# maxgillett/tinysplat

Hardware: AMD Instinct MI355X
Metric: Gaussians*pixels/s fwd+bwd (higher is better)
Workload: dtype f32; 1 GPU; 1000000 random Gaussians, SH degree 3, 1920x1080, fwd+bwd (RGB), BASELINE configs[2]; max_per_tile=614, parallelism=single GPU, tile_lists=16x16 (gsplat's) (auto), gaussian_order=as generated (i.i.d.)

## Files before the change

include/tinysplat_hip.h:

```cpp
#ifndef TINYSPLAT_HIP_H
#define TINYSPLAT_HIP_H

#include <stdint.h>

#ifdef __cplusplus
extern "C" {
#endif

#define TS_ABI_VERSION 8

#define TS_E_BADARG (-1)
#define TS_E_DEGREE (-2)

#define TS_TILE 16
#define TS_SPLAT_RECORD_FLOATS 12
#define TS_PARTIAL_ROW_FLOATS 12

int ts_abi_version(void);

typedef struct ts_camera {
    float fx, fy, cx, cy;
    int32_t img_width, img_height;
    int32_t tile_bounds_x, tile_bounds_y;
    int32_t tile_row0, tile_rows;
// ... 60 lines not shown
                    const int32_t* cum_tiles_hit, int64_t capacity, void* stream);
int ts_tile_offsets_stats(int32_t n, int32_t num_tiles, int32_t* bin_ws, int32_t* tile_bins,
                          const int32_t* cum_tiles_hit, int64_t capacity, int32_t* longest_list, void* stream);

int ts_bin_scatter(int32_t n, const float* xys, const int32_t* radii, const float* splats,
                   const ts_camera* cam_host, const int32_t* bin_ws, int32_t* bucket_ids, int32_t* scratch,
                   void* stream);

int ts_sort_tiles(int32_t num_tiles, const int32_t* tile_bins, const float* depths,
                  const int32_t* bucket_ids, int32_t* gaussian_ids_sorted, int32_t* sort_ws,
                  int32_t* zeroed_counter, void* stream);
int ts_sort_tiles_above(int32_t num_tiles, const int32_t* tile_bins, const float* depths,
                        const int32_t* bucket_ids, int32_t* gaussian_ids_sorted, int32_t* sort_ws,
                        int32_t* zeroed_counter, void* stream);

#define TS_RASTER_LOGIT_OPACITY 1

int ts_pack_splats(int32_t n, int32_t channels, int32_t flags, const float* xys, const int32_t* radii,
                   const float* conics, const float* colors, const float* opacity,
                   const int32_t* cum_tiles_hit, const ts_camera* cam_host, const float* depths,
                   float* splats, void* stream);

#define TS_RASTER_CLAMP_RGB 2
#define TS_RASTER_SPLIT_BLOCKS 4
#define TS_RASTER_NARROW_WAVES 8
#define TS_RASTER_FLAG_GEN(g) (((g) & 0xff) << 8)
int ts_raster_fwd(int32_t channels, int32_t flags, const ts_camera* cam_host, const int32_t* tile_bins,
                  const int32_t* gaussian_ids_sorted, const float* splats, const float* background,
                  float* out_img, float* final_Ts, int32_t* final_index, uint8_t* clamp_mask,
                  void* stream);
// ... 21 lines not shown

int ts_reduce_partials(int32_t n, int32_t channels, int32_t flags, const int32_t* num_tiles_hit,
                       const int32_t* cum_tiles_hit, const float* partials,
                       const uint8_t* row_flags, const float* splats, float* v_xy, float* v_conic,
                       float* v_colors, float* v_opacity, float* v_depth, const uint8_t* color_mask,
                       void* stream);

#define TS_FRAME_TIGHT 1
#define TS_FRAME_SPLIT 2
#define TS_FRAME_NARROW_WAVES 8
#define TS_FRAME_DIRECT_SCATTER 32
#define TS_FRAME_PLANES 64
#define TS_FRAME_LIST_STATS 256
#define TS_FRAME_SEPARATE_SORT 128
#define TS_FRAME_STRIPE 16
#define TS_FRAME_SURVIVORS 512
typedef struct ts_frame {
    int32_t n, num_bases, sh_degree, channels, flags;
    int32_t flag_gen;
    ts_camera cam;
    const float *means, *scales, *quats, *opacities, *colors_dc, *colors_rest;
    const float *view34, *projview, *origin, *background;
    float *xys, *depths, *conics, *colors, *splats;
    int32_t *radii, *num_tiles_hit, *cum_tiles_hit;
    uint8_t* sh_mask;
    int32_t *scan_ws, *bin_ws, *tile_bins;
    int32_t* total_host;
    int64_t num_intersects;
    int64_t capacity;
    int32_t *bucket_ids, *gaussian_ids_sorted;
// ... 285 lines not shown
```

tinysplat_amd/_lib.py:

```python
from __future__ import annotations

import ctypes
import os
from ctypes import POINTER, c_double, c_float, c_int32, c_int64, c_void_p
from pathlib import Path

LIB_PATH = Path(os.environ["TS_LIB_PATH"]) if os.environ.get("TS_LIB_PATH") else \
    Path(__file__).resolve().parent / "csrc" / "libtinysplat_hip.so"
ABI_VERSION = 8
HINT_BALANCED_WALK = 1
HINT_COOP_SPLIT = 1 << 20
PARTIAL_ROW_FLOATS = 12


class TsCamera(ctypes.Structure):
    _fields_ = [
        ("fx", c_float), ("fy", c_float), ("cx", c_float), ("cy", c_float),
        ("img_width", c_int32), ("img_height", c_int32),
        ("tile_bounds_x", c_int32), ("tile_bounds_y", c_int32),
        ("tile_row0", c_int32), ("tile_rows", c_int32),
        ("glob_scale", c_float), ("clip_thresh", c_float),
        ("wide_tiles", c_int32), ("hints", c_int32),
    ]

# ... 60 lines not shown
    "ts_project_fwd": (c_int32, [c_int32, _P, _P, _P, _P, _P, _CAM, c_int32, _P, _P, _P, _P, _P, _P, _P]),
    "ts_project_bwd": (c_int32, [c_int32, _P, _P, _P, _P, _P, _CAM, c_int32, _P, _P, _P, _P, _P, _P, _P, _P, _P]),
    "ts_sh_fwd": (c_int32, [c_int32, c_int32, c_int32, _P, _P, _P, _P]),
    "ts_sh_bwd": (c_int32, [c_int32, c_int32, c_int32, _P, _P, _P, _P]),
    "ts_sh_colors_fwd": (c_int32, [c_int32, c_int32, c_int32, _P, _P, _P, _P, _P, _P, _P, _P]),
    "ts_sh_colors_bwd": (c_int32, [c_int32, c_int32, c_int32, _P, _P, _P, _P, _P, _P, _P]),
    "ts_scan_ws_ints": (c_int64, [c_int32]),
    "ts_scan_tiles": (c_int32, [c_int32, _P, _P, _P, _P, _P]),
    "ts_bin_ws_ints": (c_int64, [c_int32, c_int32]),
    "ts_bin_count": (c_int32, [c_int32, _P, _P, _P, _CAM, _P, _P]),
    "ts_tile_offsets": (c_int32, [c_int32, c_int32, _P, _P, _P, c_int64, _P]),
    "ts_tile_offsets_stats": (c_int32, [c_int32, c_int32, _P, _P, _P, c_int64, _P, _P]),
    "ts_bin_scatter": (c_int32, [c_int32, _P, _P, _P, _CAM, _P, _P, _P, _P]),
    "ts_sort_tiles": (c_int32, [c_int32, _P, _P, _P, _P, _P, _P, _P]),
    "ts_sort_tiles_above": (c_int32, [c_int32, _P, _P, _P, _P, _P, _P, _P]),
    "ts_num_tiles": (c_int32, [_CAM]),
    "ts_final_floats": (c_int64, [_CAM, c_int32]),
    "ts_cut_tiles": (c_int32, [_CAM, _P, _P]),
    "ts_colors_pack_fwd": (c_int32, [c_int32, c_int32, c_int32, _P, _P, _P, _P, _P, _P, c_int32, c_int32,
                                     _P, _P, _P, _P, _P, _CAM, _P, _P, _P]),
    "ts_pack_splats": (c_int32, [c_int32, c_int32, c_int32, _P, _P, _P, _P, _P, _P, _CAM, _P, _P, _P]),
    "ts_raster_fwd": (c_int32, [c_int32, c_int32, _CAM, _P, _P, _P, _P, _P, _P, _P, _P, _P]),
    "ts_raster_bwd": (c_int32, [c_int32, c_int32, c_int64, _CAM, _P, _P, _P, _P, _P, _P, _P, _P, _P, _P, _P, _P]),
    "ts_raster_fwd_planes": (c_int32, [c_int32, c_int32, _CAM, _P, _P, _P, _P, _P, _P, _P, _P, _P, _P]),
    "ts_raster_fwd_sort": (c_int32, [c_int32, c_int32, _CAM, _P, _P, _P, _P, _P, _P, _P, _P, _P, _P, _P, _P]),
    "ts_raster_bwd_planes": (c_int32, [c_int32, c_int32, c_int64, _CAM, _P, _P, _P, _P, _P, _P, _P, _P, c_int32,
                                       _P, _P, _P, _P, _P]),
    "ts_bench_stream_read": (c_int32, [_P, c_int64, _P, _P]),
    "ts_bench_gather48": (c_int32, [_P, _P, c_int64, _P, _P]),
    "ts_photometric_ws_floats": (c_int64, [c_int32, c_int32]),
# ... 140 lines not shown
```

tinysplat_amd/csrc/binning.hip:

```cpp
#include <hip/hip_runtime.h>

#include "../../include/tinysplat_hip.h"
#include "host_util.h"
#include "pack.h"
#include "splat_math.h"

namespace {

constexpr int kThreads = 256;
constexpr int kScanItems = 4;
constexpr int kScanBlock = kThreads * kScanItems;

__device__ __forceinline__ int wave_inclusive_scan(int v) {
    const int lane = threadIdx.x & 63;
#pragma unroll
    for (int d = 1; d < 64; d <<= 1) {
        const int u = __shfl_up(v, d, 64);
        if (lane >= d) v += u;
    }
    return v;
}

template <int WAVES = 4>
__device__ __forceinline__ int block_inclusive_scan(int v, int* total) {
// ... 374 lines not shown
        t -= t0;
        if ((unsigned)t < (unsigned)tw) bucket_ids[atomicAdd(&cursor[t], 1)] = i;
    });
}

#ifndef TS_COARSE_SHIFT
#define TS_COARSE_SHIFT 5
#endif
constexpr int kCoarseShift = TS_COARSE_SHIFT;
constexpr int kCoarseTiles = 1 << kCoarseShift;
constexpr int kCoarseIdBits = 32 - kCoarseShift;
#ifndef TS_TWO_HOP_FROM
#define TS_TWO_HOP_FROM (1 << 18)
#endif
constexpr int kTwoHopFrom = TS_TWO_HOP_FROM;

template <bool BAL>
__global__ __launch_bounds__(kBinThreads) void bin_scatter_coarse_kernel(
    int n, int chunk, const float* __restrict__ xys, const int* __restrict__ radii,
    const float4* __restrict__ splats, const ts_camera cam, int num_tiles, const int* __restrict__ bases,
    const int* __restrict__ tile_start, int* __restrict__ scratch) {
    extern __shared__ int cursor[];
    if (tile_start[num_tiles + 1] != 0) return;
    const int groups = (num_tiles + kCoarseTiles - 1) >> kCoarseShift;
    const int* src = bases + (size_t)blockIdx.x * num_tiles;
    for (int g = threadIdx.x; g < groups; g += kBinThreads) cursor[g] = tile_start[g << kCoarseShift];
    __syncthreads();
    for (int t = threadIdx.x; t < num_tiles; t += kBinThreads) {
        const int v = src[t];
        if (v) atomicAdd(&cursor[t >> kCoarseShift], v);
    }
    __syncthreads();
    const int g0 = blockIdx.x * chunk, g1 = min(n, g0 + chunk);
    auto emit = [&](int t, int i) {
        scratch[atomicAdd(&cursor[t >> kCoarseShift], 1)] = i | ((t & (kCoarseTiles - 1)) << kCoarseIdBits);
    };
    if (BAL) walk_chunk_balanced(g0, g1, xys, radii, splats, cam, emit);
    else walk_chunk(g0, g1, xys, radii, splats, cam, emit);
}

#ifndef TS_FINE_THREADS
#define TS_FINE_THREADS 1024
#endif
#ifndef TS_FINE_AHEAD
#define TS_FINE_AHEAD 8
// ... 57 lines not shown
            }
        }
        __syncthreads();
#pragma unroll
        for (int u = 0; u < kFineAhead; ++u) {
            const int k = u * kFineThreads + (int)threadIdx.x;
            if (k < m) {
                const int t = tiles[k];
                bucket_ids[gbase[t] + (k - loff[t])] = ids[k];
            }
        }
        __syncthreads();
    }
}

constexpr int kSortCap = 4096;

#include "sort_network.h"

struct IdKeyArray {
    volatile int* ids;
    const float* depths;
};

__device__ __forceinline__ void cmpswap(IdKeyArray a, int i, int j) {
    const int x = a.ids[i], y = a.ids[j];
    if (make_key(a.depths, x) > make_key(a.depths, y)) { a.ids[i] = y; a.ids[j] = x; }
}

template <typename Ptr>
// ... 140 lines not shown
        const int s0 = start[b], m = start[b + 1] - s0;
        __syncthreads();
        if (m <= kSortCap) {
            sort_bucket_block(out + s0, depths, out + s0, m, scratch);
        } else {
            IdKeyArray a{out + s0, depths};
            bitonic_network(a, m);
        }
        __syncthreads();
    }
}

__global__ __launch_bounds__(kThreads) void sort_tiles_small_kernel(
    int num_tiles, const int* __restrict__ tile_bins, const float* __restrict__ depths,
    const int* __restrict__ bucket_ids, int* __restrict__ ids_sorted, int* __restrict__ large_count,
    int* __restrict__ large_list) {
    const int lane = threadIdx.x & 63;
    const int tile = blockIdx.x * (kThreads / 64) + (threadIdx.x >> 6);
    if (tile >= num_tiles) return;
    const int2 range = reinterpret_cast<const int2*>(tile_bins)[tile];
    const int n = range.y - range.x;
    if (n <= 0) return;
    if (n > kWaveSortMax) {
        if (n > kSortCap && lane == 0) large_list[atomicAdd(large_count, 1)] = tile;
        return;
    }
    const int* g = bucket_ids + range.x;
    int* out = ids_sorted + range.x;
    if (n <= 64) sort_tile_wave<1>(g, depths, out, n, lane);
    else if (n <= 128) sort_tile_wave<2>(g, depths, out, n, lane);
    else if (n <= 256) sort_tile_wave<4>(g, depths, out, n, lane);
// ... 18 lines not shown
    const int* __restrict__ bucket_ids, int* __restrict__ ids_sorted,
    const int* __restrict__ large_count, const int* __restrict__ large_list) {
    __shared__ unsigned long long lds_large[kLargeLdsU64];
    const int count = *large_count;
    for (int q = blockIdx.x; q < count; q += gridDim.x) {
        const int2 range = reinterpret_cast<const int2*>(tile_bins)[large_list[q]];
        const int n = range.y - range.x;
        if (n <= kSortCap) continue;
        __syncthreads();
        sort_tile_sample(bucket_ids + range.x, depths, ids_sorted + range.x, n, lds_large);
    }
}

__global__ __launch_bounds__(kThreads) void sort_tiles_above_kernel(
    const int* __restrict__ tile_bins, const float* __restrict__ depths,
    const int* __restrict__ bucket_ids, int* __restrict__ ids_sorted) {
    __shared__ unsigned long long lds_u64[kLargeLdsU64 > kSortCap / 2 ? kLargeLdsU64 : kSortCap / 2];
    const int2 range = reinterpret_cast<const int2*>(tile_bins)[blockIdx.x];
    const int n = range.y - range.x;
    if (n <= kWaveSortMax) return;
    if (n <= kSortCap) sort_bucket_block(bucket_ids + range.x, depths, ids_sorted + range.x, n, lds_u64);
    else sort_tile_sample(bucket_ids + range.x, depths, ids_sorted + range.x, n, lds_u64);
}

__global__ __launch_bounds__(kThreads) void pack_splats_kernel(int n, const ts::PackArgs a,
                                                              const float* __restrict__ colors) {
    const int i = blockIdx.x * kThreads + threadIdx.x;
    if (i >= n) return;
    if (a.radii[i] <= 0) return;
    float c0, c1, c2, c3 = 0.0f;
    if (a.channels == 4 && a.depths == nullptr) {
        const float4 c = reinterpret_cast<const float4*>(colors)[i];
// ... 71 lines not shown
    if (n < 0 || num_tiles < 0) return TS_E_BADARG;
    if (num_tiles == 0) return 0;
    if (!bin_ws || !tile_bins) return TS_E_BADARG;
    const int chunks = bin_num_chunks(n);
    int* tile_total = bin_ws + (size_t)chunks * num_tiles;
    const int per_group = (chunks + kScanGroups - 1) / kScanGroups;
    hipStream_t s = (hipStream_t)stream;
    hipLaunchKernelGGL(column_scan_kernel, dim3((num_tiles + kColTiles - 1) / kColTiles),
                       dim3(kColTiles * kScanGroups), 0, s, num_tiles, chunks, per_group, bin_ws, tile_total);
    hipLaunchKernelGGL(tile_offsets_kernel, dim3(1), dim3(kOffsetsThreads), 0, s, num_tiles, tile_total,
                       tile_bins, bin_ws + (ts_bin_ws_ints(n, num_tiles) - 1),
                       (cum_tiles_hit && n > 0) ? cum_tiles_hit + (n - 1) : nullptr, (long long)capacity, longest_list);
    return launch_status();
}

int ts_bin_scatter(int32_t n, const float* xys, const int32_t* radii, const float* splats,
                   const ts_camera* cam, const int32_t* bin_ws, int32_t* bucket_ids, int32_t* scratch,
                   void* stream) {
    if (n < 0 || !cam) return TS_E_BADARG;
    if (n == 0) return 0;
    if (!xys || !radii || !bin_ws || !bucket_ids) return TS_E_BADARG;
    const int nt = ts_num_tiles(cam);
    if (nt <= 0) return 0;
    const int chunks = bin_num_chunks(n);
    const int chunk = (n + chunks - 1) / chunks;
    const int* tile_start = bin_ws + (size_t)chunks * nt;
    if (scratch && n >= kTwoHopFrom && n < (1 << kCoarseIdBits)) {
        const int groups = (nt + kCoarseTiles - 1) >> kCoarseShift;
        if (cam->hints & TS_HINT_BALANCED_WALK)
            hipLaunchKernelGGL(bin_scatter_coarse_kernel<true>, dim3(chunks), dim3(kBinThreads),
                               (size_t)groups * sizeof(int), (hipStream_t)stream, n, chunk, xys, radii,
                               reinterpret_cast<const float4*>(splats), *cam, nt, bin_ws, tile_start, scratch);
        else
            hipLaunchKernelGGL(bin_scatter_coarse_kernel<false>, dim3(chunks), dim3(kBinThreads),
                               (size_t)groups * sizeof(int), (hipStream_t)stream, n, chunk, xys, radii,
                               reinterpret_cast<const float4*>(splats), *cam, nt, bin_ws, tile_start, scratch);
        hipLaunchKernelGGL(bin_scatter_fine_kernel, dim3(groups), dim3(kFineThreads), 0, (hipStream_t)stream, nt,
                           tile_start, scratch, bucket_ids);
        return launch_status();
    }
    const int window = bin_window_tiles(n, nt);
    const int windows = (nt + window - 1) / window;
    const size_t lds = (size_t)window * sizeof(int);
    if (lds > 64 * 1024)
        (void)hipFuncSetAttribute(reinterpret_cast<const void*>(&bin_scatter_kernel),
                                  hipFuncAttributeMaxDynamicSharedMemorySize, (int)lds);
    hipLaunchKernelGGL(bin_scatter_kernel, dim3(chunks, windows), dim3(kBinThreads), lds,
                       (hipStream_t)stream, n, chunk, xys, radii,
                       reinterpret_cast<const float4*>(splats), *cam, nt, window, bin_ws,
                       tile_start, bucket_ids);
    return launch_status();
}

int ts_sort_tiles(int32_t num_tiles, const int32_t* tile_bins, const float* depths,
                  const int32_t* bucket_ids, int32_t* gaussian_ids_sorted, int32_t* sort_ws,
                  int32_t* zeroed_counter, void* stream) {
    if (num_tiles < 0) return TS_E_BADARG;
    if (num_tiles == 0) return 0;
    if (!tile_bins || !depths || !bucket_ids || !gaussian_ids_sorted || !sort_ws) return TS_E_BADARG;
    hipStream_t s = (hipStream_t)stream;
    int32_t* counter = zeroed_counter ? zeroed_counter : sort_ws;
    int32_t* list = zeroed_counter ? sort_ws : sort_ws + 1;
    if (!zeroed_counter) {
        hipError_t e = hipMemsetAsync(sort_ws, 0, sizeof(int32_t), s);
        if (e != hipSuccess) return (int)e;
    }
    hipLaunchKernelGGL(sort_tiles_small_kernel, dim3((num_tiles + kThreads / 64 - 1) / (kThreads / 64)),
                       dim3(kThreads), 0, s, (int)num_tiles, tile_bins, depths, bucket_ids,
                       gaussian_ids_sorted, counter, list);
    hipLaunchKernelGGL(sort_tiles_mid_kernel, dim3(num_tiles), dim3(kThreads), 0, s, tile_bins, depths,
                       bucket_ids, gaussian_ids_sorted, (int*)nullptr, (int*)nullptr);
    const int grid = num_tiles < 768 ? num_tiles : 768;
    hipLaunchKernelGGL(sort_tiles_large_kernel, dim3(grid), dim3(kThreads), 0, s, tile_bins, depths,
                       bucket_ids, gaussian_ids_sorted, counter, list);
    return launch_status();
}

int ts_sort_tiles_above(int32_t num_tiles, const int32_t* tile_bins, const float* depths,
                        const int32_t* bucket_ids, int32_t* gaussian_ids_sorted, int32_t* sort_ws,
                        int32_t* zeroed_counter, void* stream) {
    if (num_tiles < 0) return TS_E_BADARG;
    if (num_tiles == 0) return 0;
    if (!tile_bins || !depths || !bucket_ids || !gaussian_ids_sorted) return TS_E_BADARG;
    (void)sort_ws; (void)zeroed_counter;
    hipLaunchKernelGGL(sort_tiles_above_kernel, dim3(num_tiles), dim3(kThreads), 0, (hipStream_t)stream, tile_bins,
                       depths, bucket_ids, gaussian_ids_sorted);
    return launch_status();
}

int ts_pack_splats(int32_t n, int32_t channels, int32_t flags, const float* xys, const int32_t* radii,
                   const float* conics, const float* colors, const float* opacity,
                   const int32_t* cum_tiles_hit, const ts_camera* cam, const float* depths, float* splats,
                   void* stream) {
    if (n < 0 || !cam || (channels != 3 && channels != 4)) return TS_E_BADARG;
    if (n == 0) return 0;
    if (!xys || !radii || !conics || !colors || !opacity || !cum_tiles_hit || !splats)
        return TS_E_BADARG;
    ts::PackArgs a;
    a.channels = channels; a.flags = (int)flags; a.xys = xys; a.radii = radii; a.conics = conics;
    a.opacity = opacity; a.cum_tiles_hit = cum_tiles_hit; a.depths = depths;
    a.splats = reinterpret_cast<float4*>(splats); a.cam = *cam;
// ... 7 lines not shown
```

tinysplat_amd/csrc/frame.hip:

```cpp
#include <hip/hip_runtime.h>

#include <atomic>
#include <cstdlib>
#if !defined(TS_NO_ROCTX) && __has_include(<rocprofiler-sdk-roctx/roctx.h>)
#include <rocprofiler-sdk-roctx/roctx.h>
#define TS_HAVE_ROCTX 1
#else
#define TS_HAVE_ROCTX 0
#endif

#include "../../include/tinysplat_hip.h"
#include "raster_survivors.h"

struct TsRange {
#if TS_HAVE_ROCTX
    explicit TsRange(const char* name) { roctxRangePush(name); }
    ~TsRange() { roctxRangePop(); }
#else
    explicit TsRange(const char*) {}
#endif
};

static std::atomic<ts_entry_probe> g_probe{nullptr};
static std::atomic<void*> g_probe_user{nullptr};
// ... 48 lines not shown
}
inline int bwd_split(const ts_frame* f) {
    return ((f->flags & TS_FRAME_SPLIT) && !segmented(f)) ? TS_RASTER_SPLIT_BLOCKS : 0;
}
inline int small_n_fused() {
    static const int v = [] {
        const char* e = getenv("TS_SMALL_N_FUSED");
        return e ? atoi(e) : 262144;
    }();
    return v;
}
inline bool survivors(const ts_frame* f) {
    return (f->flags & TS_FRAME_SURVIVORS) && f->survivors && f->final_Ts && f->num_intersects > 0 &&
           f->cam.wide_tiles == 0 &&
           !(f->flags & (TS_FRAME_SPLIT | TS_FRAME_NARROW_WAVES | TS_FRAME_SEPARATE_SORT));
}
inline int raster_flags(const ts_frame* f) {
    return TS_RASTER_CLAMP_RGB | ((f->flags & TS_FRAME_SPLIT) ? TS_RASTER_SPLIT_BLOCKS : 0) |
           ((f->flags & TS_FRAME_NARROW_WAVES) ? TS_RASTER_NARROW_WAVES : 0);
}
}

extern "C" {

int32_t ts_frame_struct_bytes(void) { return (int32_t)sizeof(ts_frame); }

int ts_set_entry_probe(ts_entry_probe fn, void* user) {
    g_probe_user.store(user, std::memory_order_relaxed);
    g_probe.store(fn, std::memory_order_release);
    return 0;
// ... 15 lines not shown
    }
    return 0;
}

int ts_frame_fwd_prepare(const ts_frame* f, void* stream) {
    TsRange range_("ts_frame_fwd_prepare");
    if (bad(f)) return TS_E_BADARG;
    TS_TRY(TS_ENTRY("ts_colors_pack_fwd",
                    ts_colors_pack_fwd(f->n, f->sh_degree, f->num_bases, f->means, f->origin, f->colors_dc,
                                       f->num_bases > 1 ? f->colors_rest : nullptr, f->sh_mask,
                                       (f->flags & TS_FRAME_STRIPE) ? f->num_tiles_hit : nullptr, f->channels,
                                       TS_RASTER_LOGIT_OPACITY, f->xys, f->radii, f->conics, f->opacities,
                                       f->cum_tiles_hit, &f->cam, f->channels == 4 ? f->depths : nullptr, f->splats,
                                       stream)));
    const float* tight = (f->flags & TS_FRAME_TIGHT) ? f->splats : nullptr;
    TS_TRY(TS_ENTRY("ts_bin_count", ts_bin_count(f->n, f->xys, f->radii, tight, &f->cam, f->bin_ws, stream)));
    int32_t* longest = nullptr;
    if ((f->flags & TS_FRAME_LIST_STATS) && f->total_host) {
        int32_t* dev = mapped_pointer(f->total_host);
        if (dev) longest = dev + 1;
    }
    TS_TRY(TS_ENTRY("ts_tile_offsets",
                    ts_tile_offsets_stats(f->n, num_tiles(f), f->bin_ws, f->tile_bins, f->cum_tiles_hit, f->capacity,
                                          longest, stream)));
    return 0;
}

int ts_frame_fwd_composite(const ts_frame* f, void* stream) {
    TsRange range_("ts_frame_fwd_composite");
    if (bad(f) || f->num_intersects < 0) return TS_E_BADARG;
    const bool planes = (f->flags & TS_FRAME_PLANES) != 0;
    if (planes && (f->channels != 4 || !f->out_depth)) return TS_E_BADARG;
    const bool fused_sort = f->num_intersects > 0 && f->cam.wide_tiles == 0 &&
                            !(f->flags & (TS_FRAME_NARROW_WAVES | TS_FRAME_SEPARATE_SORT));
    if (f->num_intersects > 0) {
        const float* tight = (f->flags & TS_FRAME_TIGHT) ? f->splats : nullptr;
        TS_TRY(TS_ENTRY("ts_bin_scatter",
                        ts_bin_scatter(f->n, f->xys, f->radii, tight, &f->cam, f->bin_ws, f->bucket_ids,
                                       (f->flags & TS_FRAME_DIRECT_SCATTER) ? nullptr : f->gaussian_ids_sorted,
                                       stream)));
        int32_t* counter = f->bin_ws + (ts_bin_ws_ints(f->n, num_tiles(f)) - 1);
        if (fused_sort)
            TS_TRY(TS_ENTRY("ts_sort_tiles",
                            ts_sort_tiles_above(num_tiles(f), f->tile_bins, f->depths, f->bucket_ids,
                                                f->gaussian_ids_sorted, f->bin_ws, counter, stream)));
        else
            TS_TRY(TS_ENTRY("ts_sort_tiles",
                            ts_sort_tiles(num_tiles(f), f->tile_bins, f->depths, f->bucket_ids, f->gaussian_ids_sorted,
                                          f->bin_ws, counter, stream)));
    }
    if (fused_sort)
        return TS_ENTRY("ts_raster_fwd",
                        ts_surv::raster_fwd_sort(f->channels, raster_flags(f), &f->cam, f->tile_bins, f->bucket_ids,
                                                 f->depths, f->gaussian_ids_sorted, f->splats, f->background,
                                                 f->out_img, planes ? f->out_depth : nullptr, f->final_Ts,
                                                 f->final_index, f->clamp_mask, survivors(f) ? f->survivors : nullptr,
                                                 stream));
    return TS_ENTRY("ts_raster_fwd",
                    ts_raster_fwd_planes(f->channels, raster_flags(f), &f->cam, f->tile_bins, f->gaussian_ids_sorted,
                                         f->splats, f->background, f->out_img, planes ? f->out_depth : nullptr,
                                         f->final_Ts, f->final_index, f->clamp_mask, stream));
}

int ts_frame_bwd_composite(const ts_frame* f, void* stream) {
// ... 185 lines not shown
```

tinysplat_amd/frame.py:

```python
from __future__ import annotations

import ctypes
import os
import threading
from typing import Optional, Tuple

import torch
import torch.distributed as dist
from torch import Tensor

from ._comm import collective_timer
from . import _lib
from ._lib import TsFrame
from .ops import TileBinning, _camera, _f32c, _need_hip, _stream, _stripe_rows, _tile_bounds, deg_from_sh

TIGHT_BINNING = os.environ.get("TS_TIGHT_BINNING", "1") != "0"

SPLIT_BLOCKS_BELOW = int(os.environ.get("TS_SPLIT_BLOCKS_BELOW", "2400"))

_ls = os.environ.get("TS_LIST_SEGMENTS", "auto")
LIST_SEGMENTS = _ls if _ls == "auto" else max(1, min(8, int(_ls)))
LIST_SEGMENTS_FROM = int(os.environ.get("TS_LIST_SEGMENTS_FROM", "192"))
SEGMENT_ITEMS = int(os.environ.get("TS_SEGMENT_ITEMS", "16384"))

# ... 128 lines not shown
        if slot[1] > 255:
            slot[0].zero_()
            slot[1] = 1
        return slot[0], slot[1]

_bg_cache = {}

STRIPE_SPARSE = os.environ.get("TS_STRIPE_SPARSE", "1") != "0"

TWO_HOP_SCATTER = os.environ.get("TS_TWO_HOP_SCATTER", "1") != "0"
INLINE_SORT = os.environ.get("TS_INLINE_SORT", "1") != "0"

DIRECT_GRADS = os.environ.get("TS_DIRECT_GRADS", "1") != "0"

SURVIVORS = os.environ.get("TS_SURVIVORS", "1") != "0"

CAPACITY_ALLOC = os.environ.get("TS_CAPACITY_ALLOC", "0") != "0"
CAPACITY_GROWTH = 1.25
_capacity = {}

COUNT_WAIT = os.environ.get("TS_COUNT_WAIT", "spin")
_SPIN_LIMIT = 50_000_000


def alloc_quantum(count: int) -> int:
    count = max(int(count), 1)
    if count <= 65536:
        return 65536
    g = 1 << (count.bit_length() - 4)
    return (count + g - 1) // g * g
# ... 100 lines not shown
        F.radii = view(5, torch.int32, n, (n,))
        F.nth = view(6, torch.int32, n, (n,))
        F.cum = view(7, torch.int32, n, (n,))
        F.tile_bins = view(10, torch.int32, 2 * max(num_tiles, 1), (max(num_tiles, 1), 2))
        host, event, count_lock = _total_slot(dev)
        fr = TsFrame()
        fr.n, fr.num_bases, fr.sh_degree, fr.channels = n, nb, int(sh_degree), ch
        stripe = STRIPE_SPARSE and cam.tile_rows < cam.tile_bounds_y
        full = cam.tile_rows == cam.tile_bounds_y
        fr.flags = ((1 if TIGHT_BINNING else 0) | (2 if F.split else 0) | (8 if mode == 2 else 0) | (16 if stripe else 0)
                    | (0 if TWO_HOP_SCATTER else 32) | (64 if F.planes else 0) | (0 if INLINE_SORT else 128)
                    | (256 if full else 0))
        surv = SURVIVORS and keep and full and mode == 0 and not F.split and INLINE_SORT
        if surv:
            fr.flags |= 512
        if full:
            _stats_mode[dev.index] = mode
        fr.cam = cam
        fr.means, fr.scales, fr.quats, fr.opacities = means.data_ptr(), scales.data_ptr(), quats.data_ptr(), opacities.data_ptr()
        fr.colors_dc, fr.colors_rest = colors_dc.data_ptr(), colors_rest.data_ptr()
        fr.view34, fr.projview, fr.origin, fr.background = view34.data_ptr(), projview.data_ptr(), origin.data_ptr(), bg.data_ptr()
        fr.splats, fr.xys, fr.conics, fr.depths = ptr[0], ptr[1], ptr[2], ptr[4]
        fr.radii, fr.num_tiles_hit, fr.cum_tiles_hit, fr.scan_ws = ptr[5], ptr[6], ptr[7], ptr[8]
        fr.bin_ws, fr.tile_bins = ptr[9], ptr[10]
        fr.total_host = host.data_ptr()
        fr.out_img = F.out_img.data_ptr()
        if F.planes:
            fr.out_depth = F.out_depth.data_ptr()
        if keep:
            fr.sh_mask, fr.final_Ts, fr.final_index, fr.clamp_mask = ptr[11], ptr[12], ptr[13], ptr[14]
# ... 242 lines not shown
```

Baseline: 2011000 billion Gaussians*pixels/s.

## Bin with per-group counts instead of per-tile counts in two-hop scatter

Adds a group-level binning path: the count kernel builds per-chunk histograms over coarse tile groups instead of every tile, a new offsets kernel scans those smaller chunk-by-group matrices, and a fine scatter kernel derives per-tile offsets and tile_bins inside each group. The longest-list statistic is now computed from per-group maxima inside the sort kernels. This cuts the size of the count workspace and the offset scan, at the cost of an extra per-group histogram pass in the fine scatter and more code paths.

```diff
diff --git a/include/tinysplat_hip.h b/include/tinysplat_hip.h
--- a/include/tinysplat_hip.h
+++ b/include/tinysplat_hip.h
@@ -98,6 +98,22 @@
                         const int32_t* bucket_ids, int32_t* gaussian_ids_sorted, int32_t* sort_ws,
                         int32_t* zeroed_counter, void* stream);
 
+int32_t ts_bin_group_form(int32_t n);
+int ts_bin_count_groups(int32_t n, const float* xys, const int32_t* radii, const float* splats,
+                        const ts_camera* cam_host, int32_t* bin_ws, void* stream);
+int ts_group_offsets(int32_t n, int32_t num_tiles, int32_t* bin_ws, int32_t* tile_bins,
+                     const int32_t* cum_tiles_hit, int64_t capacity, int32_t* longest_list, void* stream);
+int ts_bin_scatter_groups(int32_t n, const float* xys, const int32_t* radii, const float* splats,
+                          const ts_camera* cam_host, int32_t* bin_ws, int32_t* tile_bins, int32_t* bucket_ids,
+                          int32_t* scratch, void* stream);
+int ts_sort_tiles_stats(int32_t num_tiles, const int32_t* tile_bins, const float* depths,
+                        const int32_t* bucket_ids, int32_t* gaussian_ids_sorted, int32_t* sort_ws,
+                        int32_t* zeroed_counter, int32_t n, const int32_t* bin_ws, int32_t* longest_list,
+                        void* stream);
+int ts_sort_tiles_above_stats(int32_t num_tiles, const int32_t* tile_bins, const float* depths,
+                              const int32_t* bucket_ids, int32_t* gaussian_ids_sorted, int32_t n,
+                              const int32_t* bin_ws, int32_t* longest_list, void* stream);
+
 #define TS_RASTER_LOGIT_OPACITY 1
 
 int ts_pack_splats(int32_t n, int32_t channels, int32_t flags, const float* xys, const int32_t* radii,
@@ -149,6 +165,7 @@
 #define TS_FRAME_LIST_STATS 256
 #define TS_FRAME_SEPARATE_SORT 128
 #define TS_FRAME_STRIPE 16
+#define TS_FRAME_GROUP_COUNTS 1024
 #define TS_FRAME_SURVIVORS 512
 typedef struct ts_frame {
     int32_t n, num_bases, sh_degree, channels, flags;
diff --git a/tinysplat_amd/_lib.py b/tinysplat_amd/_lib.py
--- a/tinysplat_amd/_lib.py
+++ b/tinysplat_amd/_lib.py
@@ -98,6 +98,12 @@
     "ts_bin_scatter": (c_int32, [c_int32, _P, _P, _P, _CAM, _P, _P, _P, _P]),
     "ts_sort_tiles": (c_int32, [c_int32, _P, _P, _P, _P, _P, _P, _P]),
     "ts_sort_tiles_above": (c_int32, [c_int32, _P, _P, _P, _P, _P, _P, _P]),
+    "ts_bin_group_form": (c_int32, [c_int32]),
+    "ts_bin_count_groups": (c_int32, [c_int32, _P, _P, _P, _CAM, _P, _P]),
+    "ts_group_offsets": (c_int32, [c_int32, c_int32, _P, _P, _P, c_int64, _P, _P]),
+    "ts_bin_scatter_groups": (c_int32, [c_int32, _P, _P, _P, _CAM, _P, _P, _P, _P, _P]),
+    "ts_sort_tiles_stats": (c_int32, [c_int32, _P, _P, _P, _P, _P, _P, c_int32, _P, _P, _P]),
+    "ts_sort_tiles_above_stats": (c_int32, [c_int32, _P, _P, _P, _P, c_int32, _P, _P, _P]),
     "ts_num_tiles": (c_int32, [_CAM]),
     "ts_final_floats": (c_int64, [_CAM, c_int32]),
     "ts_cut_tiles": (c_int32, [_CAM, _P, _P]),
diff --git a/tinysplat_amd/csrc/binning.hip b/tinysplat_amd/csrc/binning.hip
--- a/tinysplat_amd/csrc/binning.hip
+++ b/tinysplat_amd/csrc/binning.hip
@@ -412,8 +412,110 @@
 #define TS_TWO_HOP_FROM (1 << 18)
 #endif
 constexpr int kTwoHopFrom = TS_TWO_HOP_FROM;
-
-template <bool BAL>
+inline bool two_hop(int n) { return n >= kTwoHopFrom && n < (1 << kCoarseIdBits); }
+static_assert(kTwoHopFrom >= 4096, "the group form's workspace layout needs bin_num_chunks(n) >= 4");
+
+__global__ __launch_bounds__(kBinThreads) void group_bin_count_kernel(
+    int n, int chunk, const float* __restrict__ xys, const int* __restrict__ radii,
+    const float4* __restrict__ splats, const ts_camera cam, int groups, int* __restrict__ counts) {
+    extern __shared__ int hist[];
+    for (int j = threadIdx.x; j < groups; j += kBinThreads) hist[j] = 0;
+    __syncthreads();
+    const int g0 = blockIdx.x * chunk, g1 = min(n, g0 + chunk);
+    walk_chunk(g0, g1, xys, radii, splats, cam, [&](int t, int) { atomicAdd(&hist[t >> kCoarseShift], 1); });
+    __syncthreads();
+    int* dst = counts + (size_t)blockIdx.x * groups;
+    for (int j = threadIdx.x; j < groups; j += kBinThreads) dst[j] = hist[j];
+}
+
+constexpr int kGoThreads = 1024;
+constexpr int kGoCols = 256;
+constexpr int kGoRows = kGoThreads / kGoCols;
+constexpr int kGoPer = 64;
+constexpr int kGoLdsGroups = 2048;
+constexpr int kGoSingleMax = 1 << 17;
+__global__ __launch_bounds__(kGoThreads) void group_tile_offsets_kernel(
+    int num_tiles, int groups, int chunks, int* __restrict__ counts, const int* col_total,
+    int* __restrict__ tile_start, int* __restrict__ tile_bins, int* __restrict__ spare,
+    const int* __restrict__ total_ptr, long long capacity, int* __restrict__ longest_out) {
+    __shared__ int rsum[kGoRows][kGoCols];
+    __shared__ int gtot[kGoLdsGroups];
+    __shared__ int carry, over;
+    const int tid = threadIdx.x;
+    if (tid == 0) {
+        carry = 0;
+        *spare = 0;
+        over = (total_ptr && capacity >= 0 && ((long long)*total_ptr > capacity || *total_ptr < 0)) ? 1 : 0;
+        spare[-1] = over;
+    }
+    __syncthreads();
+    if (!over) {
+        const int* tot = col_total;
+        if (counts) {
+            const int gl = tid & (kGoCols - 1), r = tid / kGoCols;
+#pragma unroll 1
+            for (int c0 = 0; c0 < groups; c0 += kGoCols) {
+                const int g = c0 + gl;
+                int colbase = 0;
+#pragma unroll 1
+                for (int r0 = 0; r0 < chunks; r0 += kGoRows * kGoPer) {
+                    const int b0 = r0 + r * kGoPer;
+                    int c[kGoPer];
+                    int sum = 0;
+                    const unsigned int col = (unsigned int)(b0 * groups + g);
+                    if (g < groups) {
+#pragma unroll
+                        for (int j = 0; j < kGoPer; ++j) c[j] = (b0 + j < chunks) ? counts[col + (unsigned int)(j * groups)] : 0;
+#pragma unroll
+                        for (int j = 0; j < kGoPer; ++j) {
+                            const int v = c[j];
+                            c[j] = sum;
+                            sum += v;
+                        }
+                    }
+                    rsum[r][gl] = sum;
+                    __syncthreads();
+                    int base = colbase, all = 0;
+#pragma unroll
+                    for (int q = 0; q < kGoRows; ++q) {
+                        const int v = rsum[q][gl];
+                        if (q < r) base += v;
+                        all += v;
+                    }
+                    if (g < groups) {
+#pragma unroll
+                        for (int j = 0; j < kGoPer; ++j)
+                            if (b0 + j < chunks) counts[col + (unsigned int)(j * groups)] = base + c[j];
+                    }
+                    colbase += all;
+                    __syncthreads();
+                }
+                if (r == 0 && g < groups) gtot[g] = colbase;
+            }
+            __syncthreads();
+            tot = gtot;
+        }
+        for (int base = 0; base < groups; base += kGoThreads) {
+            const int g = base + tid;
+            const int v = g < groups ? tot[g] : 0;
+            int total;
+            const int inc = block_inclusive_scan<kGoThreads / 64>(v, &total);
+            if (g < groups) tile_start[g << kCoarseShift] = carry + inc - v;
+            __syncthreads();
+            if (tid == 0) carry += total;
+            __syncthreads();
+        }
+        if (tid == 0) tile_start[num_tiles] = carry;
+        if (carry != 0) return;
+        if (tid == 0 && longest_out) *longest_out = 0;
+    }
+    for (int t = tid; t <= num_tiles; t += kGoThreads) {
+        tile_start[t] = 0;
+        if (t < num_tiles) reinterpret_cast<int2*>(tile_bins)[t] = make_int2(0, 0);
+    }
+}
+
+template <bool BAL, bool GROUPS = false>
 __global__ __launch_bounds__(kBinThreads) void bin_scatter_coarse_kernel(
     int n, int chunk, const float* __restrict__ xys, const int* __restrict__ radii,
     const float4* __restrict__ splats, const ts_camera cam, int num_tiles, const int* __restrict__ bases,
@@ -421,12 +523,17 @@
     extern __shared__ int cursor[];
     if (tile_start[num_tiles + 1] != 0) return;
     const int groups = (num_tiles + kCoarseTiles - 1) >> kCoarseShift;
-    const int* src = bases + (size_t)blockIdx.x * num_tiles;
-    for (int g = threadIdx.x; g < groups; g += kBinThreads) cursor[g] = tile_start[g << kCoarseShift];
-    __syncthreads();
-    for (int t = threadIdx.x; t < num_tiles; t += kBinThreads) {
-        const int v = src[t];
-        if (v) atomicAdd(&cursor[t >> kCoarseShift], v);
+    if (GROUPS) {
+        const int* src = bases + (size_t)blockIdx.x * groups;
+        for (int g = threadIdx.x; g < groups; g += kBinThreads) cursor[g] = tile_start[g << kCoarseShift] + src[g];
+    } else {
+        const int* src = bases + (size_t)blockIdx.x * num_tiles;
+        for (int g = threadIdx.x; g < groups; g += kBinThreads) cursor[g] = tile_start[g << kCoarseShift];
+        __syncthreads();
+        for (int t = threadIdx.x; t < num_tiles; t += kBinThreads) {
+            const int v = src[t];
+            if (v) atomicAdd(&cursor[t >> kCoarseShift], v);
+        }
     }
     __syncthreads();
     const int g0 = blockIdx.x * chunk, g1 = min(n, g0 + chunk);
@@ -514,6 +621,142 @@
     }
 }
 
+__global__ __launch_bounds__(kFineThreads) void bin_scatter_fine_groups_kernel(int num_tiles,
+                                                                               int* __restrict__ tile_start,
+                                                                               int* __restrict__ tile_bins,
+                                                                               int* __restrict__ group_max,
+                                                                               const int* __restrict__ scratch,
+                                                                               int* __restrict__ bucket_ids) {
+    if (tile_start[num_tiles + 1] != 0) return;
+    __shared__ int cursor[kCoarseTiles];
+    const int t0 = blockIdx.x << kCoarseShift, t1 = min(num_tiles, t0 + kCoarseTiles);
+    const int begin = tile_start[t0], end = tile_start[t1];
+    __shared__ int hist[kCoarseTiles], loff[kCoarseTiles + 1], gbase[kCoarseTiles];
+    __shared__ int ids[kFinePass];
+    __shared__ unsigned char tiles[kFinePass];
+    if ((int)threadIdx.x < kCoarseTiles) {
+        hist[threadIdx.x] = 0;
+        cursor[threadIdx.x] = 0;
+    }
+    __syncthreads();
+    auto publish = [&](int t, int c, int ex) {
+        const int s = begin + ex;
+        if (t < t1 - t0) {
+            cursor[t] = s;
+            if (t > 0) tile_start[t0 + t] = s;
+            reinterpret_cast<int2*>(tile_bins)[t0 + t] = c > 0 ? make_int2(s, s + c) : make_int2(0, 0);
+        }
+        int longest = c;
+#pragma unroll
+        for (int d = 32; d >= 1; d >>= 1) longest = max(longest, __shfl_xor(longest, d, 64));
+        if (t == 0) group_max[blockIdx.x] = longest;
+    };
+    const bool counted = end - begin > kFinePass || end == begin;
+    if (counted) {
+        for (int c0 = begin; c0 < end; c0 += kFinePass) {
+            const int m = min(kFinePass, end - c0);
+            unsigned int w[kFineAhead];
+#pragma unroll
+            for (int u = 0; u < kFineAhead; ++u) {
+                const int k = u * kFineThreads + (int)threadIdx.x;
+                if (k < m) w[u] = (unsigned int)scratch[c0 + k];
+            }
+#pragma unroll
+            for (int u = 0; u < kFineAhead; ++u) {
+                const int k = u * kFineThreads + (int)threadIdx.x;
+                if (k < m) atomicAdd(&hist[w[u] >> kCoarseIdBits], 1);
+            }
+        }
+        __syncthreads();
+        if ((int)threadIdx.x < 64) {
+            const int t = threadIdx.x;
+            const int c = t < kCoarseTiles ? hist[t] : 0;
+            int inc = c;
+#pragma unroll
+            for (int d = 1; d < kCoarseTiles; d <<= 1) {
+                const int o = __shfl_up(inc, d, 64);
+                if (t >= d) inc += o;
+            }
+            publish(t, c, inc - c);
+            if (t < kCoarseTiles) hist[t] = 0;
+        }
+        __syncthreads();
+    }
+    for (int c0 = begin; c0 < end; c0 += kFinePass) {
+        const int m = min(kFinePass, end - c0);
+        unsigned int w[kFineAhead];
+        int rank[kFineAhead];
+#pragma unroll
+        for (int u = 0; u < kFineAhead; ++u) {
+            const int k = u * kFineThreads + (int)threadIdx.x;
+            if (k < m) w[u] = (unsigned int)scratch[c0 + k];
+        }
+#pragma unroll
+        for (int u = 0; u < kFineAhead; ++u) {
+            const int k = u * kFineThreads + (int)threadIdx.x;
+            if (k < m) rank[u] = atomicAdd(&hist[w[u] >> kCoarseIdBits], 1);
+        }
+        __syncthreads();
+        if ((int)threadIdx.x < 64) {
+            const int t = threadIdx.x;
+            const int c = t < kCoarseTiles ? hist[t] : 0;
+            int inc = c;
+#pragma unroll
+            for (int d = 1; d < kCoarseTiles; d <<= 1) {
+                const int o = __shfl_up(inc, d, 64);
+                if (t >= d) inc += o;
+            }
+            if (!counted) publish(t, c, inc - c);
+            if (t < kCoarseTiles) {
+                loff[t] = inc - c;
+                gbase[t] = cursor[t];
+                cursor[t] += c;
+                hist[t] = 0;
+            }
+        }
+        __syncthreads();
+#pragma unroll
+        for (int u = 0; u < kFineAhead; ++u) {
+            const int k = u * kFineThreads + (int)threadIdx.x;
+            if (k < m) {
+                const int t = (int)(w[u] >> kCoarseIdBits);
+                const int lp = loff[t] + rank[u];
+                ids[lp] = (int)(w[u] & ((1u << kCoarseIdBits) - 1u));
+                tiles[lp] = (unsigned char)t;
+            }
+        }
+        __syncthreads();
+#pragma unroll
+        for (int u = 0; u < kFineAhead; ++u) {
+            const int k = u * kFineThreads + (int)threadIdx.x;
+            if (k < m) {
+                const int t = tiles[k];
+                bucket_ids[gbase[t] + (k - loff[t])] = ids[k];
+            }
+        }
+        __syncthreads();
+    }
+}
+
+struct ListStats {
+    const int* group_max;
+    const int* guard;
+    int* longest_out;
+    int groups;
+};
+__device__ __forceinline__ void store_longest(const ListStats& st) {
+    __shared__ int longest;
+    if (threadIdx.x == 0) longest = 0;
+    __syncthreads();
+    int m = 0;
+    for (int g = threadIdx.x; g < st.groups; g += kThreads) m = max(m, st.group_max[g]);
+#pragma unroll
+    for (int d = 32; d >= 1; d >>= 1) m = max(m, __shfl_xor(m, d, 64));
+    if ((threadIdx.x & 63) == 0) atomicMax(&longest, m);
+    __syncthreads();
+    if (threadIdx.x == 0 && *st.guard == 0) *st.longest_out = longest;
+}
+
 constexpr int kSortCap = 4096;
 
 #include "sort_network.h"
@@ -684,7 +927,8 @@
 __global__ __launch_bounds__(kThreads) void sort_tiles_small_kernel(
     int num_tiles, const int* __restrict__ tile_bins, const float* __restrict__ depths,
     const int* __restrict__ bucket_ids, int* __restrict__ ids_sorted, int* __restrict__ large_count,
-    int* __restrict__ large_list) {
+    int* __restrict__ large_list, const ListStats stats) {
+    if (stats.group_max && blockIdx.x == 0) store_longest(stats);
     const int lane = threadIdx.x & 63;
     const int tile = blockIdx.x * (kThreads / 64) + (threadIdx.x >> 6);
     if (tile >= num_tiles) return;
@@ -733,8 +977,9 @@
 
 __global__ __launch_bounds__(kThreads) void sort_tiles_above_kernel(
     const int* __restrict__ tile_bins, const float* __restrict__ depths,
-    const int* __restrict__ bucket_ids, int* __restrict__ ids_sorted) {
+    const int* __restrict__ bucket_ids, int* __restrict__ ids_sorted, const ListStats stats) {
     __shared__ unsigned long long lds_u64[kLargeLdsU64 > kSortCap / 2 ? kLargeLdsU64 : kSortCap / 2];
+    if (stats.group_max && blockIdx.x == 0) store_longest(stats);
     const int2 range = reinterpret_cast<const int2*>(tile_bins)[blockIdx.x];
     const int n = range.y - range.x;
     if (n <= kWaveSortMax) return;
@@ -836,6 +1081,76 @@
     return launch_status();
 }
 
+int32_t ts_bin_group_form(int32_t n) { return two_hop(n) ? 1 : 0; }
+
+int ts_bin_count_groups(int32_t n, const float* xys, const int32_t* radii, const float* splats,
+                        const ts_camera* cam, int32_t* bin_ws, void* stream) {
+    if (!cam || !bin_ws || !xys || !radii || !two_hop(n)) return TS_E_BADARG;
+    const int nt = ts_num_tiles(cam);
+    if (nt <= 0) return 0;
+    const int chunks = bin_num_chunks(n);
+    const int chunk = (n + chunks - 1) / chunks;
+    const int groups = (nt + kCoarseTiles - 1) >> kCoarseShift;
+    hipLaunchKernelGGL(group_bin_count_kernel, dim3(chunks), dim3(kBinThreads), (size_t)groups * sizeof(int),
+                       (hipStream_t)stream, n, chunk, xys, radii, reinterpret_cast<const float4*>(splats), *cam,
+                       groups, bin_ws);
+    return launch_status();
+}
+
+int ts_group_offsets(int32_t n, int32_t num_tiles, int32_t* bin_ws, int32_t* tile_bins,
+                     const int32_t* cum_tiles_hit, int64_t capacity, int32_t* longest_list, void* stream) {
+    if (num_tiles < 0 || !two_hop(n)) return TS_E_BADARG;
+    if (num_tiles == 0) return 0;
+    if (!bin_ws || !tile_bins) return TS_E_BADARG;
+    const int chunks = bin_num_chunks(n);
+    const int groups = (num_tiles + kCoarseTiles - 1) >> kCoarseShift;
+    int* tile_start = bin_ws + (size_t)chunks * num_tiles;
+    int* spare = bin_ws + (ts_bin_ws_ints(n, num_tiles) - 1);
+    const int* total_ptr = cum_tiles_hit ? cum_tiles_hit + (n - 1) : nullptr;
+    hipStream_t s = (hipStream_t)stream;
+    if ((long long)chunks * groups <= kGoSingleMax && groups <= kGoLdsGroups) {
+        hipLaunchKernelGGL(group_tile_offsets_kernel, dim3(1), dim3(kGoThreads), 0, s, num_tiles, groups, chunks,
+                           bin_ws, (const int*)nullptr, tile_start, tile_bins, spare, total_ptr, (long long)capacity,
+                           longest_list);
+    } else {
+        int* col_total = bin_ws + (size_t)chunks * groups;
+        const int per_group = (chunks + kScanGroups - 1) / kScanGroups;
+        hipLaunchKernelGGL(column_scan_kernel, dim3((groups + kColTiles - 1) / kColTiles),
+                           dim3(kColTiles * kScanGroups), 0, s, groups, chunks, per_group, bin_ws, col_total);
+        hipLaunchKernelGGL(group_tile_offsets_kernel, dim3(1), dim3(kGoThreads), 0, s, num_tiles, groups, chunks,
+                           (int*)nullptr, (const int*)col_total, tile_start, tile_bins, spare, total_ptr,
+                           (long long)capacity, longest_list);
+    }
+    return launch_status();
+}
+
+int ts_bin_scatter_groups(int32_t n, const float* xys, const int32_t* radii, const float* splats,
+                          const ts_camera* cam, int32_t* bin_ws, int32_t* tile_bins, int32_t* bucket_ids,
+                          int32_t* scratch, void* stream) {
+    if (!cam || !xys || !radii || !bin_ws || !tile_bins || !bucket_ids || !scratch || !two_hop(n))
+        return TS_E_BADARG;
+    const int nt = ts_num_tiles(cam);
+    if (nt <= 0) return 0;
+    const int chunks = bin_num_chunks(n);
+    const int chunk = (n + chunks - 1) / chunks;
+    const int groups = (nt + kCoarseTiles - 1) >> kCoarseShift;
+    int* tile_start = bin_ws + (size_t)chunks * nt;
+    hipStream_t s = (hipStream_t)stream;
+    if (cam->hints & TS_HINT_BALANCED_WALK)
+        hipLaunchKernelGGL((bin_scatter_coarse_kernel<true, true>), dim3(chunks), dim3(kBinThreads),
+                           (size_t)groups * sizeof(int), s, n, chunk, xys, radii,
+                           reinterpret_cast<const float4*>(splats), *cam, nt, (const int*)bin_ws,
+                           (const int*)tile_start, scratch);
+    else
+        hipLaunchKernelGGL((bin_scatter_coarse_kernel<false, true>), dim3(chunks), dim3(kBinThreads),
+                           (size_t)groups * sizeof(int), s, n, chunk, xys, radii,
+                           reinterpret_cast<const float4*>(splats), *cam, nt, (const int*)bin_ws,
+                           (const int*)tile_start, scratch);
+    hipLaunchKernelGGL(bin_scatter_fine_groups_kernel, dim3(groups), dim3(kFineThreads), 0, s, nt, tile_start,
+                       tile_bins, bin_ws + nt + 1, (const int*)scratch, bucket_ids);
+    return launch_status();
+}
+
 int ts_bin_scatter(int32_t n, const float* xys, const int32_t* radii, const float* splats,
                    const ts_camera* cam, const int32_t* bin_ws, int32_t* bucket_ids, int32_t* scratch,
                    void* stream) {
@@ -847,7 +1162,7 @@
     const int chunks = bin_num_chunks(n);
     const int chunk = (n + chunks - 1) / chunks;
     const int* tile_start = bin_ws + (size_t)chunks * nt;
-    if (scratch && n >= kTwoHopFrom && n < (1 << kCoarseIdBits)) {
+    if (scratch && two_hop(n)) {
         const int groups = (nt + kCoarseTiles - 1) >> kCoarseShift;
         if (cam->hints & TS_HINT_BALANCED_WALK)
             hipLaunchKernelGGL(bin_scatter_coarse_kernel<true>, dim3(chunks), dim3(kBinThreads),
@@ -874,12 +1189,39 @@
     return launch_status();
 }
 
+}
+
+namespace {
+inline bool list_stats(int n, int num_tiles, const int32_t* bin_ws, int32_t* longest_list, ListStats* st) {
+    *st = ListStats{nullptr, nullptr, nullptr, 0};
+    if (!longest_list) return true;
+    if (!bin_ws || !two_hop(n) || num_tiles <= 0) return false;
+    st->group_max = bin_ws + num_tiles + 1;
+    st->guard = bin_ws + (size_t)bin_num_chunks(n) * num_tiles + num_tiles + 1;
+    st->longest_out = longest_list;
+    st->groups = (num_tiles + kCoarseTiles - 1) >> kCoarseShift;
+    return true;
+}
+}
+
+extern "C" {
+
 int ts_sort_tiles(int32_t num_tiles, const int32_t* tile_bins, const float* depths,
                   const int32_t* bucket_ids, int32_t* gaussian_ids_sorted, int32_t* sort_ws,
                   int32_t* zeroed_counter, void* stream) {
+    return ts_sort_tiles_stats(num_tiles, tile_bins, depths, bucket_ids, gaussian_ids_sorted, sort_ws, zeroed_counter,
+                               0, nullptr, nullptr, stream);
+}
+
+int ts_sort_tiles_stats(int32_t num_tiles, const int32_t* tile_bins, const float* depths,
+                        const int32_t* bucket_ids, int32_t* gaussian_ids_sorted, int32_t* sort_ws,
+                        int32_t* zeroed_counter, int32_t n, const int32_t* bin_ws, int32_t* longest_list,
+                        void* stream) {
     if (num_tiles < 0) return TS_E_BADARG;
     if (num_tiles == 0) return 0;
     if (!tile_bins || !depths || !bucket_ids || !gaussian_ids_sorted || !sort_ws) return TS_E_BADARG;
+    ListStats stats;
+    if (!list_stats(n, num_tiles, bin_ws, longest_list, &stats)) return TS_E_BADARG;
     hipStream_t s = (hipStream_t)stream;
     int32_t* counter = zeroed_counter ? zeroed_counter : sort_ws;
     int32_t* list = zeroed_counter ? sort_ws : sort_ws + 1;
@@ -889,7 +1231,7 @@
     }
     hipLaunchKernelGGL(sort_tiles_small_kernel, dim3((num_tiles + kThreads / 64 - 1) / (kThreads / 64)),
                        dim3(kThreads), 0, s, (int)num_tiles, tile_bins, depths, bucket_ids,
-                       gaussian_ids_sorted, counter, list);
+                       gaussian_ids_sorted, counter, list, stats);
     hipLaunchKernelGGL(sort_tiles_mid_kernel, dim3(num_tiles), dim3(kThreads), 0, s, tile_bins, depths,
                        bucket_ids, gaussian_ids_sorted, (int*)nullptr, (int*)nullptr);
     const int grid = num_tiles < 768 ? num_tiles : 768;
@@ -901,12 +1243,21 @@
 int ts_sort_tiles_above(int32_t num_tiles, const int32_t* tile_bins, const float* depths,
                         const int32_t* bucket_ids, int32_t* gaussian_ids_sorted, int32_t* sort_ws,
                         int32_t* zeroed_counter, void* stream) {
+    (void)sort_ws; (void)zeroed_counter;
+    return ts_sort_tiles_above_stats(num_tiles, tile_bins, depths, bucket_ids, gaussian_ids_sorted, 0, nullptr, nullptr,
+                                     stream);
+}
+
+int ts_sort_tiles_above_stats(int32_t num_tiles, const int32_t* tile_bins, const float* depths,
+                              const int32_t* bucket_ids, int32_t* gaussian_ids_sorted, int32_t n,
+                              const int32_t* bin_ws, int32_t* longest_list, void* stream) {
     if (num_tiles < 0) return TS_E_BADARG;
     if (num_tiles == 0) return 0;
     if (!tile_bins || !depths || !bucket_ids || !gaussian_ids_sorted) return TS_E_BADARG;
-    (void)sort_ws; (void)zeroed_counter;
+    ListStats stats;
+    if (!list_stats(n, num_tiles, bin_ws, longest_list, &stats)) return TS_E_BADARG;
     hipLaunchKernelGGL(sort_tiles_above_kernel, dim3(num_tiles), dim3(kThreads), 0, (hipStream_t)stream, tile_bins,
-                       depths, bucket_ids, gaussian_ids_sorted);
+                       depths, bucket_ids, gaussian_ids_sorted, stats);
     return launch_status();
 }
 
diff --git a/tinysplat_amd/csrc/frame.hip b/tinysplat_amd/csrc/frame.hip
--- a/tinysplat_amd/csrc/frame.hip
+++ b/tinysplat_amd/csrc/frame.hip
@@ -86,6 +86,16 @@
     return (f->flags & TS_FRAME_SURVIVORS) && f->survivors && f->final_Ts && f->num_intersects > 0 &&
            f->cam.wide_tiles == 0 &&
            !(f->flags & (TS_FRAME_SPLIT | TS_FRAME_NARROW_WAVES | TS_FRAME_SEPARATE_SORT));
+}
+inline bool group_counts(const ts_frame* f) {
+    return (f->flags & TS_FRAME_GROUP_COUNTS) && !(f->flags & TS_FRAME_DIRECT_SCATTER) && ts_bin_group_form(f->n);
+}
+inline int32_t* longest_word(const ts_frame* f) {
+    if ((f->flags & TS_FRAME_LIST_STATS) && f->total_host) {
+        int32_t* dev = mapped_pointer(f->total_host);
+        if (dev) return dev + 1;
+    }
+    return nullptr;
 }
 inline int raster_flags(const ts_frame* f) {
     return TS_RASTER_CLAMP_RGB | ((f->flags & TS_FRAME_SPLIT) ? TS_RASTER_SPLIT_BLOCKS : 0) |
@@ -131,12 +141,15 @@
                                        f->cum_tiles_hit, &f->cam, f->channels == 4 ? f->depths : nullptr, f->splats,
                                        stream)));
     const float* tight = (f->flags & TS_FRAME_TIGHT) ? f->splats : nullptr;
+    int32_t* longest = longest_word(f);
+    if (group_counts(f)) {
+        TS_TRY(TS_ENTRY("ts_bin_count",
+                        ts_bin_count_groups(f->n, f->xys, f->radii, tight, &f->cam, f->bin_ws, stream)));
+        return TS_ENTRY("ts_tile_offsets",
+                        ts_group_offsets(f->n, num_tiles(f), f->bin_ws, f->tile_bins, f->cum_tiles_hit, f->capacity,
+                                         longest, stream));
+    }
     TS_TRY(TS_ENTRY("ts_bin_count", ts_bin_count(f->n, f->xys, f->radii, tight, &f->cam, f->bin_ws, stream)));
-    int32_t* longest = nullptr;
-    if ((f->flags & TS_FRAME_LIST_STATS) && f->total_host) {
-        int32_t* dev = mapped_pointer(f->total_host);
-        if (dev) longest = dev + 1;
-    }
     TS_TRY(TS_ENTRY("ts_tile_offsets",
                     ts_tile_offsets_stats(f->n, num_tiles(f), f->bin_ws, f->tile_bins, f->cum_tiles_hit, f->capacity,
                                           longest, stream)));
@@ -152,19 +165,27 @@
                             !(f->flags & (TS_FRAME_NARROW_WAVES | TS_FRAME_SEPARATE_SORT));
     if (f->num_intersects > 0) {
         const float* tight = (f->flags & TS_FRAME_TIGHT) ? f->splats : nullptr;
-        TS_TRY(TS_ENTRY("ts_bin_scatter",
-                        ts_bin_scatter(f->n, f->xys, f->radii, tight, &f->cam, f->bin_ws, f->bucket_ids,
-                                       (f->flags & TS_FRAME_DIRECT_SCATTER) ? nullptr : f->gaussian_ids_sorted,
-                                       stream)));
+        const bool groups = group_counts(f);
+        if (groups)
+            TS_TRY(TS_ENTRY("ts_bin_scatter",
+                            ts_bin_scatter_groups(f->n, f->xys, f->radii, tight, &f->cam, f->bin_ws, f->tile_bins,
+                                                  f->bucket_ids, f->gaussian_ids_sorted, stream)));
+        else
+            TS_TRY(TS_ENTRY("ts_bin_scatter",
+                            ts_bin_scatter(f->n, f->xys, f->radii, tight, &f->cam, f->bin_ws, f->bucket_ids,
+                                           (f->flags & TS_FRAME_DIRECT_SCATTER) ? nullptr : f->gaussian_ids_sorted,
+                                           stream)));
         int32_t* counter = f->bin_ws + (ts_bin_ws_ints(f->n, num_tiles(f)) - 1);
+        int32_t* longest = groups ? longest_word(f) : nullptr;
         if (fused_sort)
             TS_TRY(TS_ENTRY("ts_sort_tiles",
-                            ts_sort_tiles_above(num_tiles(f), f->tile_bins, f->depths, f->bucket_ids,
-                                                f->gaussian_ids_sorted, f->bin_ws, counter, stream)));
+                            ts_sort_tiles_above_stats(num_tiles(f), f->tile_bins, f->depths, f->bucket_ids,
+                                                      f->gaussian_ids_sorted, f->n, f->bin_ws, longest, stream)));
         else
             TS_TRY(TS_ENTRY("ts_sort_tiles",
-                            ts_sort_tiles(num_tiles(f), f->tile_bins, f->depths, f->bucket_ids, f->gaussian_ids_sorted,
-                                          f->bin_ws, counter, stream)));
+                            ts_sort_tiles_stats(num_tiles(f), f->tile_bins, f->depths, f->bucket_ids,
+                                                f->gaussian_ids_sorted, f->bin_ws, counter, f->n, f->bin_ws, longest,
+                                                stream)));
     }
     if (fused_sort)
         return TS_ENTRY("ts_raster_fwd",
diff --git a/tinysplat_amd/frame.py b/tinysplat_amd/frame.py
--- a/tinysplat_amd/frame.py
+++ b/tinysplat_amd/frame.py
@@ -166,6 +166,8 @@
 DIRECT_GRADS = os.environ.get("TS_DIRECT_GRADS", "1") != "0"
 
 SURVIVORS = os.environ.get("TS_SURVIVORS", "1") != "0"
+
+GROUP_COUNTS = os.environ.get("TS_GROUP_COUNTS", "1") != "0"
 
 CAPACITY_ALLOC = os.environ.get("TS_CAPACITY_ALLOC", "0") != "0"
 CAPACITY_GROWTH = 1.25
@@ -296,6 +298,8 @@
         surv = SURVIVORS and keep and full and mode == 0 and not F.split and INLINE_SORT
         if surv:
             fr.flags |= 512
+        if GROUP_COUNTS:
+            fr.flags |= 1024
         if full:
             _stats_mode[dev.index] = mode
         fr.cam = cam
```

Measured after the change: 2042000 billion Gaussians*pixels/s (median of 6 runs). 1.6% higher.
